# totgokhung123/Event-Retrival-In-Video-Learning-Transferable-Visual-Model-From-Supervised-Natural-Language

Measured on AMD Instinct MI355X. Metric: frames/sec embedded+ranked, ViT-B/32 224², 1/2/4/8 MI355X; R@1/5/10 parity, higher is better.
Workload: dtype bf16; 1 GPU; ViT-B/32 bf16, 10000 frames/GPU x 32 text queries, top-10 (BASELINE configs[1]); frames_per_gpu=10000, global_frames=10000, queries=32, k=10, image_chunk=10000, parallelism=dp1

## Files before the change

### event-retrival-in-video-learning-transferable-visual-model-from-supervised-natural-language_amd/csrc/api.cpp

```cpp
#include <hip/hip_runtime.h>

#include <cmath>
#include <cstdarg>
#include <cstdlib>
#include <cstdio>
#include <cstring>
#include <algorithm>
#include <functional>
#include <memory>
#include <mutex>
#include <string>
#include <system_error>
#include <thread>
#include <vector>

#include "../../include/miclip.h"
#include "src_hash.h"
#include "internal.hpp"

using namespace miclip;

namespace {

thread_local std::string g_err;
// ... 1405 lines not shown

int mi_op_split2h(const float* x, int64_t ldx, int64_t rows, int32_t K, int32_t role, int32_t gelu, void* out,
                  float* scale, void* stream) {
  if (!x || !out || !scale || rows < 0 || role < 0 || role > 2 || (gelu & ~1))
    return fail(MI_ERR_ARG, "mi_op_split2h: bad arguments");
  if (K < 4 || K > 4096 || K % 4 || ldx < K || ldx % 4)
    return fail(MI_ERR_UNSUPPORTED, "mi_op_split2h: 4 <= K <= 4096, K %% 4 == 0, ldx >= K, ldx %% 4 == 0");
  HIP_TRY(split2h_rows(x, ldx, rows, K, role, gelu, (uint16_t*)out, scale, (hipStream_t)stream));
  return MI_OK;
}

int mi_op_gemm_split2h(const void* A3, const void* W3, const float* a_scale, const float* w_scale, const float* bias,
                       float* out, int32_t M, int32_t N, int32_t K3, int32_t epi, void* stream) {
  const int dup = (epi >> 8) & 1;
  epi &= ~0x100;
  if (!A3 || !W3 || !a_scale || !w_scale || !out || M < 0 || N < 1 || K3 < 1 || (epi != EPI_F32 && epi != EPI_RESID_F32))
    return fail(MI_ERR_ARG, "mi_op_gemm_split2h: bad arguments");
  if (N % 128 || K3 % 32) return fail(MI_ERR_UNSUPPORTED, "mi_op_gemm_split2h: N %% 128 == 0, K3 %% 32 == 0");
  GemmArgs g = gargs((const uint16_t*)A3, dup ? 2 * (K3 / 3) : K3, (const uint16_t*)W3, K3, bias, out, N, M, N, K3);
  g.variant = 0;
  g.a_f16 = 1;
  g.rsc = a_scale;
  g.csc = w_scale;
  g.a_dup = dup ? K3 / 3 : 0;
  if (dup && (K3 % 3 || !bias || !gemm_8q_ok(g)))
    return fail(MI_ERR_UNSUPPORTED, "mi_op_gemm_split2h: the [x1 x2] layout needs M >= 256, N %% 256 == 0, K %% 64 == 0");
  HIP_TRY(gemm_bf16(g, epi, (hipStream_t)stream));
  return MI_OK;
}

int mi_op_attention_f32_split(const float* qkv, const float* rmax, float bw, float bb, void* out, int32_t role,
                              float* scale, int32_t B, int32_t S, int32_t W, int32_t causal, void* stream) {
  if (!qkv || !rmax || !out || !scale || B < 0 || S < 1 || W < 64 || (causal & ~1) || (role != 0 && role != 2))
    return fail(MI_ERR_ARG, "mi_op_attention_f32_split: bad arguments");
  if (W % 64 || S > 64) return fail(MI_ERR_UNSUPPORTED, "mi_op_attention_f32_split: W %% 64 == 0 and S <= 64");
  HIP_TRY(attention_f32_split(qkv, rmax, bw, bb, (uint16_t*)out, role, scale, B, S, W, causal, (hipStream_t)stream));
  return MI_OK;
}

int mi_op_attention_f32(const float* qkv, float* out, int32_t B, int32_t S, int32_t W, int32_t causal, void* stream) {
  if (!qkv || !out || B < 0 || S < 1 || W < 64 || (causal & ~1)) return fail(MI_ERR_ARG, "mi_op_attention_f32: bad arguments");
  if (W % 64) return fail(MI_ERR_UNSUPPORTED, "mi_op_attention_f32: W %% 64 == 0");
  HIP_TRY(attention_f32(qkv, out, B, S, W, causal, (hipStream_t)stream));
  return MI_OK;
}

int mi_op_residual_stats(void* x, const void* delta, float* rs, int32_t rows, int32_t W, void* stream) {
  if (!x || !delta || !rs || rows < 0) return fail(MI_ERR_ARG, "mi_op_residual_stats: bad arguments");
  if (W % 4 || W > 1024) return fail(MI_ERR_UNSUPPORTED, "mi_op_residual_stats: W must be a multiple of 4, <= 1024");
  HIP_TRY(residual_stats((float*)x, (const uint16_t*)delta, rs, rows, W, (hipStream_t)stream));
  return MI_OK;
}

int mi_op_gemm_ln(const void* x16, int64_t lda, const float* rs, const void* wf, const float* colsum,
                  const float* colc, void* out, int32_t M, int32_t N, int32_t K, int32_t gelu, void* stream) {
  if (!x16 || !rs || !wf || !colsum || !colc || !out || M < 0 || (gelu & ~1))
    return fail(MI_ERR_ARG, "mi_op_gemm_ln: bad arguments");
  if (M == 0) return MI_OK;
  GemmArgs g = gargs((const uint16_t*)x16, lda, (const uint16_t*)wf, K, colc, out, N, M, N, K);
  g.variant = 0;
  g.a_f16 = 1;
  g.rs = rs;
  g.colv = colsum;
  if (lda < K || lda % 8 || !gemm_8q_ok(g))
    return fail(MI_ERR_UNSUPPORTED, "mi_op_gemm_ln: needs N %% 256 == 0, K %% 128 == 0, K >= 256, M >= 256, "
                                    "lda >= K with lda %% 8 == 0");
  HIP_TRY(gemm_bf16(g, gelu ? EPI_LN_GELU_BF16 : EPI_LN_BF16, (hipStream_t)stream));
  return MI_OK;
}

int mi_op_gemm_residual(void* x16, int64_t ldx, const void* A, int64_t lda, const void* w, const float* bias,
                        float* ps, float* rs, int32_t M, int32_t W, int32_t K, void* stream) {
  if (!x16 || !A || !w || !ps || !rs || M < 0) return fail(MI_ERR_ARG, "mi_op_gemm_residual: bad arguments");
  if (M == 0) return MI_OK;
  GemmArgs g = gargs((const uint16_t*)A, lda, (const uint16_t*)w, K, bias, x16, ldx, M, W, K);
  g.ps = ps;
  if (lda < K || lda % 8 || ldx < W || ldx % 8 || W > 1024 || ((uintptr_t)x16 & 15) || !gemm_8q_ok(g))
    return fail(MI_ERR_UNSUPPORTED, "mi_op_gemm_residual: needs W %% 256 == 0, W <= 1024, K %% 128 == 0, K >= 256, "
                                    "M >= 256, lda >= K and ldx >= W multiples of 8, x16 16-byte aligned");
  HIP_TRY(gemm_bf16(g, EPI_RES16_BF16, (hipStream_t)stream));
  HIP_TRY(residual_finalize(ps, rs, M, W, (hipStream_t)stream));
  return MI_OK;
}

int mi_op_attention(const void* qkv, void* out, int32_t B, int32_t S, int32_t W, int32_t causal, void* stream) {
  if (!qkv || !out || B < 0 || S < 1) return fail(MI_ERR_ARG, "mi_op_attention: bad arguments");
  if (W % 64 || S > 640 || (causal & ~(ATT_CAUSAL | ATT_ONE_WAVE | ATT_STREAM))) return fail(MI_ERR_UNSUPPORTED, "mi_op_attention: W %% 64 == 0 and S <= 640");
  if ((causal & ATT_ONE_WAVE) && !MICLIP_AB) return fail(MI_ERR_UNSUPPORTED, "mi_op_attention: the one-wave kernel (bit 8) is in the A/B build");
  HIP_TRY(attention((const uint16_t*)qkv, (uint16_t*)out, B, S, W, causal, (hipStream_t)stream));
  return MI_OK;
}

int mi_op_gemm_mx(const void* A, const void* a_scale, const void* W, const void* w_scale, const float* bias, void* out,
                  int32_t M, int32_t N, int32_t K, int32_t epi, void* stream) {
  if (!A || !W || !a_scale || !w_scale || !out || M < 0) return fail(MI_ERR_ARG, "mi_op_gemm_mx: bad arguments");
  if (K % 128 || N % 256 || K <= 0) return fail(MI_ERR_UNSUPPORTED, "mi_op_gemm_mx: needs K %% 128 == 0, N %% 256 == 0");
  const int variant = epi >> 8;
  if (variant && !MICLIP_AB) return fail(MI_ERR_UNSUPPORTED, "mi_op_gemm_mx: kernel overrides need the A/B build (make ab)");
  epi &= 0xff;
  if (epi != 0 && epi != 1 && epi != 3 && epi != 4)
    return fail(MI_ERR_ARG, "mi_op_gemm_mx: epilogue 0 (bf16), 1 (GELU), 3 (f32) or 4 (GELU -> MX-fp8)");
  GemmArgs g = gargs((const uint16_t*)A, K, (const uint16_t*)W, K, bias, out, N, M, N, K);
  g.variant = variant;
  g.a_scale = (const uint8_t*)a_scale;
  g.w_scale = (const uint8_t*)w_scale;
  if (epi == 4) g.o_scale = (uint8_t*)out + ((int64_t)M * N + 255) / 256 * 256;
  HIP_TRY(gemm_mx(g, epi, (hipStream_t)stream));
  return MI_OK;
}

int mi_op_quantize_mx(const void* in, void* q, void* scales, int32_t rows, int32_t K, void* stream) {
  if (!in || !q || !scales || rows < 0) return fail(MI_ERR_ARG, "mi_op_quantize_mx: bad arguments");
  if (K % 128 || K <= 0) return fail(MI_ERR_UNSUPPORTED, "mi_op_quantize_mx: K %% 128 == 0");
  HIP_TRY(quantize_mx((const uint16_t*)in, K, (uint8_t*)q, K, (uint8_t*)scales, rows, K, (hipStream_t)stream));
  return MI_OK;
}

int mi_resample_coeffs(int32_t in_size, double in0, double in1, int32_t out_size, int filter, int32_t* kk,
                       int64_t kk_cap, int32_t* bounds) {
  if (!kk || !bounds || in_size < 1 || out_size < 1 || (filter != MI_RESAMPLE_BICUBIC && filter != MI_RESAMPLE_BILINEAR))
    return fail(MI_ERR_ARG, "mi_resample_coeffs: bad arguments");
  std::vector<int32_t> k, b;
  const int ks = resample_coeffs(in_size, in0, in1, out_size, filter, k, b);
  if (ks < 0) return fail(MI_ERR_ARG, "mi_resample_coeffs: bad arguments");
  if ((int64_t)k.size() > kk_cap) return fail(MI_ERR_ARG, "mi_resample_coeffs: kk needs %zu entries", k.size());
  memcpy(kk, k.data(), k.size() * 4);
  memcpy(bounds, b.data(), b.size() * 4);
  return ks;
}

size_t mi_preprocess_workspace_bytes(int64_t B, int32_t H, int32_t W, int32_t n, int mode) {
  return preprocess_workspace_bytes(B, H, W, n, mode);
}

int mi_preprocess_frames(const uint8_t* frames, int64_t B, int32_t H, int32_t W, int32_t n, int mode, void* out,
                         int out_dtype, void* workspace, size_t workspace_bytes, void* stream) {
  if (B < 0 || H < 1 || W < 1 || n < 1 || n > 4096) return fail(MI_ERR_ARG, "mi_preprocess_frames: bad sizes");
  if (mode != MI_PREP_CLIP && mode != MI_PREP_SQUASH) return fail(MI_ERR_ARG, "mi_preprocess_frames: bad mode");
  if (out_dtype != MI_F32 && out_dtype != MI_BF16) return fail(MI_ERR_ARG, "mi_preprocess_frames: out_dtype f32/bf16");
  if (B == 0) return MI_OK;
// ... 115 lines not shown
```

### event-retrival-in-video-learning-transferable-visual-model-from-supervised-natural-language_amd/csrc/attention.hip

```cpp
#include <algorithm>
#include <cstdlib>
#include <type_traits>

#include "common.hpp"
#include "internal.hpp"

namespace miclip {

namespace {


typedef short s16x4 __attribute__((ext_vector_type(4)));
typedef short s16x8 __attribute__((ext_vector_type(8)));

template <int V>
using Int = std::integral_constant<int, V>;

constexpr float sl2 = 0.125f * 1.4426950408889634f;
constexpr float RESCALE = 8.0f;

template <bool P16 = true>
__device__ __forceinline__ float group_max(float v) {
  if (P16) {
    const auto a = __builtin_amdgcn_permlane16_swap(__float_as_uint(v), __float_as_uint(v), false, false);
// ... 314 lines not shown
      }
      const float mu = m[t];
      float ps[4];
#pragma unroll
      for (int kt = 0; kt < 4; ++kt) {
#pragma unroll
        for (int j = 0; j < 4; ++j) sc[kt][j] = __builtin_amdgcn_exp2f(fmaf(sc[kt][j], sl2, -mu));
        ps[kt] = (sc[kt][0] + sc[kt][1]) + (sc[kt][2] + sc[kt][3]);
      }
      l[t] += (ps[0] + ps[1]) + (ps[2] + ps[3]);
      if (SLOTS == 1) {
        __builtin_amdgcn_sched_barrier(0);
        read_vf();
        if (VB) asm volatile("s_waitcnt lgkmcnt(0)" ::: "memory");
      }
#pragma unroll
      for (int s = 0; s < 2; ++s) {
        if (s == 1 && kvalid <= 32) break;
        bf16x8 pb;
#pragma unroll
        for (int j = 0; j < 4; ++j) {
          pb[j] = (__bf16)sc[2 * s][j];
          pb[4 + j] = (__bf16)sc[2 * s + 1][j];
        }
#pragma unroll
        for (int dt = 0; dt < 4; ++dt) o[t][dt] = __builtin_amdgcn_mfma_f32_16x16x32_bf16(vf[dt][s], pb, o[t][dt], 0, 0, 0);
      }
    }
    if (SLOTS > 1 && c + 1 < nch) FA_STAGE_WRITE(slot ^ 1);
    __syncthreads();
  }
#undef FA_STAGE_LOAD
#undef FA_STAGE_WRITE

#pragma unroll
  for (int t = 0; t < NT; ++t) {
    const int qt = wave + NW * t;
    if (qt >= nqt) continue;
    AttnOut{out, q8, qs, rows_pad, bseq, S, W, h}.store16(qt * 16 + fr, g, o[t], 1.0f / group_sum(l[t]));
  }
  if (!PIPE) break;
  item += (int)gridDim.x;
  if (item >= items) break;
  first = false;
  }
}

template <int NT, int PP, int SLOTS = 2>
__global__ __launch_bounds__(512) void attention_flash_kernel(const uint16_t* __restrict__ qkv,
                                                                uint16_t* __restrict__ out, int S, int W, int H,
                                                                int causal, uint8_t* __restrict__ q8,
                                                                uint8_t* __restrict__ qs, int64_t rows_pad) {
  attention_flash_body<NT, PP, SLOTS>(qkv, out, S, W, H, causal, q8, qs, rows_pad);
}

#if MICLIP_AB
__global__ __launch_bounds__(256) __attribute__((amdgpu_waves_per_eu(6))) void attention_short_kernel(
    const uint16_t* __restrict__ qkv, uint16_t* __restrict__ out, int S, int W, int H, int causal,
    uint8_t* __restrict__ q8, uint8_t* __restrict__ qs, int64_t rows_pad) {
  attention_flash_body<1, 2, 1>(qkv, out, S, W, H, causal, q8, qs, rows_pad);
}

__global__ __launch_bounds__(256) void attention_pipe_kernel(const uint16_t* __restrict__ qkv, uint16_t* __restrict__ out,
                                                             int S, int W, int H, int causal, uint8_t* __restrict__ q8,
                                                             uint8_t* __restrict__ qs, int64_t rows_pad, int items) {
  attention_flash_body<1, 2, 1, 1, true>(qkv, out, S, W, H, causal, q8, qs, rows_pad, items);
}

__global__ __launch_bounds__(256) void attention_vb_kernel(const uint16_t* __restrict__ qkv, uint16_t* __restrict__ out,
                                                           int S, int W, int H, int causal, uint8_t* __restrict__ q8,
                                                           uint8_t* __restrict__ qs, int64_t rows_pad) {
  attention_flash_body<1, 2, 1, 1, false, true>(qkv, out, S, W, H, causal, q8, qs, rows_pad);
}

__global__ __launch_bounds__(512) __attribute__((amdgpu_waves_per_eu(6))) void attention_short2_kernel(
    const uint16_t* __restrict__ qkv, uint16_t* __restrict__ out, int S, int W, int H, int causal,
    uint8_t* __restrict__ q8, uint8_t* __restrict__ qs, int64_t rows_pad) {
  attention_flash_body<1, 2, 1, 2>(qkv, out, S, W, H, causal, q8, qs, rows_pad);
}
#endif


template <int NW, bool TT2 = true, bool SPLIT = false, bool SFIRST = false, bool QPF = false>
__global__ __launch_bounds__(NW * 64) void attention_res_kernel(const uint16_t* __restrict__ qkv,
                                                                uint16_t* __restrict__ out, int S, int W, int H,
                                                                uint8_t* __restrict__ q8, uint8_t* __restrict__ qs,
                                                                int64_t rows_pad) {
  extern __shared__ __attribute__((aligned(16))) char res_lds[];
  const int spad = (S + 31) & ~31;
  char* Kimg = res_lds;
  char* Vimg = res_lds + spad * 128;
  const int item = blockIdx.x;
  const int bseq = item / H, h = item % H;
  const int tid = threadIdx.x, lane = tid & 63;
  const int wave = __builtin_amdgcn_readfirstlane(tid >> 6);
  const int64_t ld = 3 * (int64_t)W;
  const uint16_t* qb = qkv + (int64_t)bseq * S * ld + h * 64;
  const uint16_t* kb = qb + W;
  const uint16_t* vb = qb + 2 * W;

  {
    const int nr8 = spad >> 3;
    const int slot = lane & 7;
    for (int i = wave; i < 2 * nr8; i += NW) {
      const bool isv = i >= nr8;
      const int i8 = isv ? i - nr8 : i;
// ... 483 lines not shown
      case 3:
        return launch_kernel(attention_short_kernel, items, 256, s, qkv, out, S, W, H, causal, q8, qs, rows_pad);
      case 1:
        if (!causal)
          return launch_kernel<attention_res_kernel<4, false>>(items, 256, res_lds, s, qkv, out, S, W, H, q8, qs, rows_pad);
        break;
      default: break;
    }
  }
#endif

  if (!one_wave && !stream && !causal && S > 64) {
    int var = ab_env_int("MICLIP_ATTN_VAR", 0);
    if (var < 1 || var > 14) var = S > 320 ? 5 : 1;
    const int vr = S - 16 * ((S + 15) / 16 - 1);
    if (var == 11 || ((var == 12 || var == 13) && !(vr <= 4 && !q8))) var = 1;
    auto res = [&](auto k, int threads, size_t lds) {
      return launch_kernel<decltype(k)::value>(items, threads, lds, s, qkv, out, S, W, H, q8, qs, rows_pad);
    };
    auto r32 = [&](auto k, int threads, int stagger_ticks) {
      return launch_kernel<decltype(k)::value>(items, threads, res_lds, s, qkv, out, S, W, H, q8, qs, rows_pad,
                                               stagger_ticks);
    };
    switch (var) {
      case 1: return res(Kern<attention_res_kernel<8, false>>{}, 512, res_lds);
      case 5: return r32(Kern<attention_r32_kernel<12, false>>{}, 768, 0);
#if MICLIP_AB
      case 2: return res(Kern<attention_res_kernel<8, true>>{}, 512, res_lds);
      case 3: return res(Kern<attention_res_kernel<16, false>>{}, 1024, res_lds);
      case 4: return r32(Kern<attention_r32_kernel<8, true>>{}, 512, 0);
      case 6:
      case 7:
        return r32(Kern<attention_r32_kernel<12, false>>{}, 768, (var - 5) * (S * S / 378));
      case 8: return r32(Kern<attention_r32_kernel<12, false, 2>>{}, 768, 0);
      case 10: return r32(Kern<attention_r32_kernel<12, false, 0, true>>{}, 768, 0);
      case 12: return res(Kern<attention_res_kernel<8, false, true>>{}, 512, res_lds + (size_t)8 * vr * 68 * 4);
      case 13: return res(Kern<attention_res_kernel<8, false, true, true>>{}, 512, res_lds + (size_t)8 * vr * 68 * 4);
      case 14: return res(Kern<attention_res_kernel<8, false, false, false, true>>{}, 512, res_lds);
      default: return r32(Kern<attention_r32_kernel<12, false, 1>>{}, 768, 0);
#else
      default: return hipErrorNotSupported;
#endif
    }
  }

#if MICLIP_AB
  if (one_wave)
    return with_value<32, 64, 96>(std::max(32, (S + 31) & ~31), [&](auto sp) {
      return launch_kernel(attention_kernel<decltype(sp)::value>, items, 64, s, qkv, out, S, W, H, causal, items);
    });
#endif

  const int nqt = (S + 15) / 16;
  if (nqt <= 4)
    return launch_kernel(attention_flash_kernel<1, 2, 1>, items, 256, s, qkv, out, S, W, H, causal | q0, q8, qs, rows_pad);
  return with_value<1, 2, 3, 4, 5>((nqt + 7) / 8, [&](auto nt) {
    return launch_kernel(attention_flash_kernel<decltype(nt)::value, 1>, items, 512, s, qkv, out, S, W, H, causal, q8, qs,
                         rows_pad);
  });
}

}
```

### event-retrival-in-video-learning-transferable-visual-model-from-supervised-natural-language_amd/csrc/encoder.hip

```cpp
#include <cstdlib>

#include "common.hpp"
#include "internal.hpp"

namespace miclip {

namespace {

constexpr float LN_EPS = 1e-5f;

struct RowVals {
  float4 v[4];
};

__device__ __forceinline__ void ln_stats(RowVals& r, int n4, int lane, int W, float& mean, float& rstd) {
  float s = 0.f;
#pragma unroll
  for (int i = 0; i < 4; ++i)
    if (lane + 64 * i < n4) s += (r.v[i].x + r.v[i].y) + (r.v[i].z + r.v[i].w);
  mean = wave_sum(s) / (float)W;
  float ss = 0.f;
#pragma unroll
  for (int i = 0; i < 4; ++i)
    if (lane + 64 * i < n4) {
// ... 108 lines not shown
  float mean, rstd;
  ln_stats(r, n4, lane, W, mean, rstd);
  ln_store(r, mean, rstd, g, b, out + (int64_t)row * W, q, qs, row, (rows + 1) & ~1, lane, n4);
}

__global__ __launch_bounds__(256) void vision_embed_ln_kernel(float* __restrict__ x, const float* __restrict__ cls,
                                                              const float* __restrict__ pos, const float* __restrict__ g,
                                                              const float* __restrict__ b, int rows, int S, int W,
                                                              const float* __restrict__ g1,
                                                              const float* __restrict__ b1, uint16_t* __restrict__ h) {
  const int row = blockIdx.x * 4 + (threadIdx.x >> 6), lane = threadIdx.x & 63;
  if (row >= rows) return;
  const int t = row % S, n4 = W >> 2;
  float4* xr = (float4*)(x + (int64_t)row * W);
  const float4* src = t == 0 ? (const float4*)cls : (const float4*)xr;
  const float4* p4 = (const float4*)(pos + (int64_t)t * W);
  RowVals r;
#pragma unroll
  for (int i = 0; i < 4; ++i) {
    const int idx = lane + 64 * i;
    if (idx < n4) {
      const float4 s = src[idx], p = p4[idx];
      r.v[i] = make_float4(s.x + p.x, s.y + p.y, s.z + p.z, s.w + p.w);
    } else {
      r.v[i] = make_float4(0.f, 0.f, 0.f, 0.f);
    }
  }
  float mean, rstd;
  ln_stats(r, n4, lane, W, mean, rstd);
  const float4* g4 = (const float4*)g;
  const float4* b4 = (const float4*)b;
#pragma unroll
  for (int i = 0; i < 4; ++i) {
    const int idx = lane + 64 * i;
    if (idx < n4) {
      const float4 gg = g4[idx], bb = b4[idx];
      r.v[i] = make_float4((r.v[i].x - mean) * rstd * gg.x + bb.x, (r.v[i].y - mean) * rstd * gg.y + bb.y,
                           (r.v[i].z - mean) * rstd * gg.z + bb.z, (r.v[i].w - mean) * rstd * gg.w + bb.w);
      xr[idx] = r.v[i];
    }
  }
  if (h) {
    ln_stats(r, n4, lane, W, mean, rstd);
    ln_store(r, mean, rstd, g1, b1, h + (int64_t)row * W, nullptr, nullptr, row, 0, lane, n4);
  }
}

__device__ __forceinline__ void store_row_stats(RowVals& r, int n4, int lane, int W, float* rs, int row) {
  float mean, rstd;
  ln_stats(r, n4, lane, W, mean, rstd);
  if (lane == 0) *(float2*)(rs + 2 * (int64_t)row) = make_float2(rstd, rstd * mean);
}

__global__ __launch_bounds__(256) void vision_embed_ln16_kernel(float* __restrict__ x, const float* __restrict__ cls,
                                                                const float* __restrict__ pos,
                                                                const float* __restrict__ g,
                                                                const float* __restrict__ b, int rows, int S, int W,
                                                                float* __restrict__ rs) {
  typedef _Float16 h4v __attribute__((ext_vector_type(4)));
  const int row = blockIdx.x * 4 + (threadIdx.x >> 6), lane = threadIdx.x & 63;
  if (row >= rows) return;
  const int t = row % S, n4 = W >> 2;
  const float4* xr = (const float4*)(x + (int64_t)row * W);
  h4v* xh = (h4v*)((_Float16*)x + (int64_t)row * W * 2);
  const float4* src = t == 0 ? (const float4*)cls : xr;
  const float4* p4 = (const float4*)(pos + (int64_t)t * W);
  RowVals r;
#pragma unroll
  for (int i = 0; i < 4; ++i) {
    const int idx = lane + 64 * i;
    if (idx < n4) {
      const float4 sv = src[idx], p = p4[idx];
      r.v[i] = make_float4(sv.x + p.x, sv.y + p.y, sv.z + p.z, sv.w + p.w);
    } else {
      r.v[i] = make_float4(0.f, 0.f, 0.f, 0.f);
    }
  }
  float mean, rstd;
  ln_stats(r, n4, lane, W, mean, rstd);
  const float4* g4 = (const float4*)g;
  const float4* b4 = (const float4*)b;
#pragma unroll
  for (int i = 0; i < 4; ++i) {
    const int idx = lane + 64 * i;
    if (idx < n4) {
      const float4 gg = g4[idx], bb = b4[idx];
      const h4v o{(_Float16)((r.v[i].x - mean) * rstd * gg.x + bb.x), (_Float16)((r.v[i].y - mean) * rstd * gg.y + bb.y),
                  (_Float16)((r.v[i].z - mean) * rstd * gg.z + bb.z), (_Float16)((r.v[i].w - mean) * rstd * gg.w + bb.w)};
      r.v[i] = make_float4((float)o[0], (float)o[1], (float)o[2], (float)o[3]);
      xh[idx] = o;
    }
  }
  store_row_stats(r, n4, lane, W, rs, row);
}

__global__ __launch_bounds__(256) void residual_stats_kernel(float* __restrict__ x, const uint16_t* __restrict__ delta,
                                                             float* __restrict__ rs, int rows, int W) {
  typedef _Float16 h4v __attribute__((ext_vector_type(4)));
  typedef uint32_t u2v __attribute__((ext_vector_type(2)));
  const int row = blockIdx.x * 4 + (threadIdx.x >> 6), lane = threadIdx.x & 63;
  if (row >= rows) return;
  const int n4 = W >> 2;
  h4v* xh = (h4v*)((_Float16*)x + (int64_t)row * W * 2);
  const u2v* dr = (const u2v*)(delta + (int64_t)row * W);
  RowVals r;
#pragma unroll
  for (int i = 0; i < 4; ++i) {
    const int idx = lane + 64 * i;
    if (idx < n4) {
      const h4v vh = __builtin_nontemporal_load(&xh[idx]);
      const u2v d = __builtin_nontemporal_load(&dr[idx]);
      const h4v o{(_Float16)((float)vh[0] + bf2f((uint16_t)(d[0] & 0xffff))),
                  (_Float16)((float)vh[1] + bf2f((uint16_t)(d[0] >> 16))),
                  (_Float16)((float)vh[2] + bf2f((uint16_t)(d[1] & 0xffff))),
                  (_Float16)((float)vh[3] + bf2f((uint16_t)(d[1] >> 16)))};
      __builtin_nontemporal_store(o, &xh[idx]);
      r.v[i] = make_float4((float)o[0], (float)o[1], (float)o[2], (float)o[3]);
    } else {
      r.v[i] = make_float4(0.f, 0.f, 0.f, 0.f);
    }
  }
  store_row_stats(r, n4, lane, W, rs, row);
}

__global__ __launch_bounds__(256) void residual_finalize_kernel(const float* __restrict__ ps, float* __restrict__ rs,
                                                                int rows, int W) {
  __shared__ float4 sp[256 * 8 + 256 / 4];
  const int np = W >> 6, nq = np >> 1;
  const int r0 = blockIdx.x * 256;
  const int nrow = min(256, rows - r0);
  const float4* src = (const float4*)(ps + (int64_t)r0 * np * 2);
  for (int i = threadIdx.x; i < nrow * nq; i += 256) {
    const int r = i / nq;
    sp[i + (r >> 2)] = src[i];
  }
  __syncthreads();
  const int row = r0 + threadIdx.x;
  if (row >= rows) return;
  const float4* p4 = sp + threadIdx.x * nq + (threadIdx.x >> 2);
  float s[16], m2[16];
#pragma unroll
  for (int i = 0; i < 8; ++i)
    if (i < nq) {
// ... 142 lines not shown
      }
    }
    packed[e >> 1] = (uint32_t)f2bf(v[0]) | ((uint32_t)f2bf(v[1]) << 16);
  }
  *(uint4*)(out + prow * Kp + kb) = make_uint4(packed[0], packed[1], packed[2], packed[3]);
}

__global__ __launch_bounds__(256) void finalize_kernel(const float* __restrict__ y, void* __restrict__ out,
                                                       int out_dtype, int rows, int D, int l2) {
  const int row = blockIdx.x * 4 + (threadIdx.x >> 6), lane = threadIdx.x & 63;
  if (row >= rows) return;
  const float* yr = y + (int64_t)row * D;
  float inv = 1.f;
  if (l2) {
    float ss = 0.f;
    for (int c = lane; c < D; c += 64) ss += yr[c] * yr[c];
    const float n = sqrtf(wave_sum(ss));
    inv = (l2 == 2 && !(n > 1e-8f)) ? 1.0f : 1.0f / n;
  }
  for (int c = lane; c < D; c += 64) {
    const float v = l2 ? yr[c] * inv : yr[c];
    if (out_dtype == 0) ((float*)out)[(int64_t)row * D + c] = v;
    else if (out_dtype == 1) ((uint16_t*)out)[(int64_t)row * D + c] = f2bf(v);
    else ((_Float16*)out)[(int64_t)row * D + c] = (_Float16)v;
  }
}

}

hipError_t layernorm_bf16(const float* x, int64_t in_stride, const float* g, const float* b, uint16_t* out,
                          int64_t out_stride, int rows, int W, hipStream_t s, uint8_t* q, uint8_t* qs) {
  if (rows <= 0) return hipSuccess;
  if (W % 4 || W > 1024 || (q && W % 128)) return hipErrorInvalidValue;
  hipLaunchKernelGGL(ln_bf16_kernel, dim3((rows + 3) / 4), dim3(256), 0, s, x, in_stride, g, b, out, out_stride,
                     rows, W, q, qs);
  return hipGetLastError();
}

hipError_t vision_embed_ln(float* x, const float* cls, const float* pos, const float* g, const float* b, int B,
                           int S, int W, hipStream_t s, const float* g1, const float* b1, uint16_t* h) {
  const int rows = B * S;
  if (rows <= 0) return hipSuccess;
  if (W % 4 || W > 1024) return hipErrorInvalidValue;
  hipLaunchKernelGGL(vision_embed_ln_kernel, dim3((rows + 3) / 4), dim3(256), 0, s, x, cls, pos, g, b, rows, S, W,
                     g1, b1, h);
  return hipGetLastError();
}

hipError_t vision_embed_ln16(float* x, const float* cls, const float* pos, const float* g, const float* b, int B,
                             int S, int W, float* rs, hipStream_t s) {
  const int rows = B * S;
  if (W % 4 || W > 1024) return hipErrorInvalidValue;
  if (rows <= 0) return hipSuccess;
  hipLaunchKernelGGL(vision_embed_ln16_kernel, dim3((rows + 3) / 4), dim3(256), 0, s, x, cls, pos, g, b, rows, S, W, rs);
  return hipGetLastError();
}

hipError_t residual_stats(float* x, const uint16_t* delta, float* rs, int rows, int W, hipStream_t s) {
  if (W % 4 || W > 1024) return hipErrorInvalidValue;
  if (rows <= 0) return hipSuccess;
  hipLaunchKernelGGL(residual_stats_kernel, dim3((rows + 3) / 4), dim3(256), 0, s, x, delta, rs, rows, W);
  return hipGetLastError();
}

hipError_t residual_finalize(const float* ps, float* rs, int rows, int W, hipStream_t s) {
  if (W % 128 || W > 1024 || W <= 0) return hipErrorInvalidValue;
  if (rows <= 0) return hipSuccess;
  hipLaunchKernelGGL(residual_finalize_kernel, dim3((rows + 255) / 256), dim3(256), 0, s, ps, rs, rows, W);
  return hipGetLastError();
}

hipError_t text_embed(const int32_t* tokens, const float* tok_emb, const float* pos, float* x, int Q, int S, int W,
                      int vocab, hipStream_t s) {
  const int64_t total4 = (int64_t)Q * S * (W / 4);
  if (total4 <= 0) return hipSuccess;
  hipLaunchKernelGGL(text_embed_kernel, dim3((unsigned)((total4 + 255) / 256)), dim3(256), 0, s, tokens, tok_emb,
                     pos, x, total4, S, W, vocab);
  return hipGetLastError();
}

hipError_t eot_gather_ln(const int32_t* tokens, const float* x, const uint16_t* delta, const float* g,
                         const float* b, uint16_t* out, int Q, int S, int W, hipStream_t s) {
  if (Q <= 0) return hipSuccess;
  hipLaunchKernelGGL(eot_gather_ln_kernel, dim3((Q + 3) / 4), dim3(256), 0, s, tokens, x, delta, g, b, out, Q, S,
                     W);
  return hipGetLastError();
}

hipError_t residual_ln(float* x, const uint16_t* delta, int64_t stride, int write_x, const float* g, const float* b,
                       uint16_t* out, int rows, int W, hipStream_t s, uint8_t* q, uint8_t* qs, int xmode) {
  if (rows <= 0) return hipSuccess;
  if (W % 4 || W > 1024 || (q && W % 128) || xmode < RES_F32 || xmode > RES_F16) return hipErrorInvalidValue;
#if MICLIP_AB
  static int nts = -1;
  if (nts < 0) {
    const char* e = getenv("MICLIP_LN_NT");
    nts = e ? atoi(e) : 1;
  }
#else
  constexpr int nts = 1;
#endif
  const dim3 grid((rows + 3) / 4), block(256);
#define RLN(NT, XM) hipLaunchKernelGGL((residual_ln_kernel<NT, XM>), grid, block, 0, s, x, delta, stride, write_x, g, b, out, rows, W, q, qs)
  if (nts) {
    if (xmode == RES_F32) RLN(true, RES_F32);
    else if (xmode == RES_F32_TO_F16) RLN(true, RES_F32_TO_F16);
    else RLN(true, RES_F16);
  } else {
// ... 35 lines not shown
```

### event-retrival-in-video-learning-transferable-visual-model-from-supervised-natural-language_amd/miclip/_native.py

```python
from __future__ import annotations

import ctypes
import os

import numpy as np

from .config import CLIPConfig

LIB_NAME = "libmiclip.so"
LIB_PATH = os.path.join(os.path.dirname(os.path.abspath(__file__)), LIB_NAME)
CSRC_DIR = os.path.join(os.path.dirname(os.path.dirname(os.path.abspath(__file__))), "csrc")
AB_LIB_PATH = os.path.join(os.path.dirname(os.path.dirname(os.path.dirname(os.path.abspath(__file__)))),
                           "scripts", "ab", "libmiclip_ab.so")

MI_F32, MI_BF16, MI_F16, MI_FP8 = 0, 1, 2, 3
MI_NAN_FIRST, MI_NAN_LAST = 0, 1
MI_NORM_L2, MI_NORM_L2_GUARD, MI_NORM_NONE = 0, 1, 2
MI_PREP_CLIP, MI_PREP_SQUASH = 0, 1
MI_RESAMPLE_BICUBIC, MI_RESAMPLE_BILINEAR = 0, 1

EXPORTS = (
    "mi_abi_version", "mi_build_id", "mi_build_sources", "mi_last_error", "mi_clip_weights_numel", "mi_clip_create", "mi_clip_destroy",
    "mi_clip_reserve", "mi_clip_encode_image", "mi_clip_encode_text", "mi_rank_workspace_bytes",
    "mi_rank_topk", "mi_rank_merge", "mi_score_matrix", "mi_rank_of_targets",
    "mi_op_gemm", "mi_op_gemm_f32", "mi_op_layernorm", "mi_op_attention", "mi_op_residual_ln",
    "mi_op_residual_stats", "mi_op_gemm_ln", "mi_op_gemm_residual", "mi_op_split6",
    "mi_resample_coeffs", "mi_preprocess_workspace_bytes", "mi_preprocess_frames",
    "mi_jpeg_workspace_bytes", "mi_jpeg_decode", "mi_host_gather",
    "mi_op_quantize_mx", "mi_op_gemm_mx",
    "mi_mirror_build", "mi_rank_mirror_workspace_bytes", "mi_rank_mirror", "mi_normalize_rows_f16",
    "mi_jpeg_decode_transform", "mi_op_split2h", "mi_op_gemm_split2h", "mi_op_attention_f32",
    "mi_op_attention_f32_split",
    "mi_clip_kernel_events", "mi_clip_kernel_times",
    "mi_rank_filtered_workspace_bytes", "mi_rank_topk_filtered",
    "mi_rank_collapse_workspace_bytes", "mi_rank_collapse",
)


class MiClipError(RuntimeError):
    pass


class Arch(ctypes.Structure):
    _fields_ = [(n, ctypes.c_int32) for n in (
        "embed_dim", "image_resolution", "vision_layers", "vision_width", "vision_patch_size",
        "context_length", "vocab_size", "text_width", "text_heads", "text_layers")]

    @classmethod
    def from_config(cls, cfg: CLIPConfig) -> "Arch":
        return cls(cfg.embed_dim, cfg.image_resolution, cfg.vision_layers, cfg.vision_width,
                   cfg.vision_patch_size, cfg.context_length, cfg.vocab_size, cfg.text_width,
                   cfg.text_heads, cfg.text_layers)


_lib = None
_lib_ab = None


def lib():
    global _lib
    if _lib is not None:
        return _lib
    if os.environ.get("MICLIP_LIB") == "ab":
        _lib = lib_ab()
        return _lib
    if not os.path.isfile(LIB_PATH):
        raise MiClipError(f"{LIB_PATH} not found: build it with `python -c 'import __graft_entry__ as g; g.build()'`"
                          " or `make -C <pkg>/csrc`")
    _lib = _bind(LIB_PATH)
    return _lib


def lib_ab():
    global _lib_ab
    if _lib_ab is not None:
        return _lib_ab
    if not os.path.isfile(AB_LIB_PATH):
        raise MiClipError(f"{AB_LIB_PATH} not found: `make -C <pkg>/csrc ab`")
    _lib_ab = _bind(AB_LIB_PATH)
    return _lib_ab


def _bind(path):
    import torch
    L = ctypes.CDLL(path)
    P, I32, I64, SZ = ctypes.c_void_p, ctypes.c_int32, ctypes.c_int64, ctypes.c_size_t
    sig = {
        "mi_abi_version": (ctypes.c_int, []),
        "mi_build_id": (ctypes.c_char_p, []),
        "mi_build_sources": (ctypes.c_char_p, []),
        "mi_last_error": (ctypes.c_char_p, []),
        "mi_clip_weights_numel": (I64, [ctypes.POINTER(Arch)]),
        "mi_clip_create": (ctypes.c_int, [ctypes.POINTER(Arch), P, I64, ctypes.c_int, ctypes.c_int,
                                          ctypes.POINTER(P)]),
        "mi_clip_destroy": (ctypes.c_int, [P]),
        "mi_clip_reserve": (ctypes.c_int, [P, I64, I64]),
        "mi_clip_encode_image": (ctypes.c_int, [P, P, I64, ctypes.c_int, P, ctypes.c_int, ctypes.c_int, P]),
        "mi_clip_encode_text": (ctypes.c_int, [P, P, I64, P, ctypes.c_int, ctypes.c_int, P]),
        "mi_rank_workspace_bytes": (SZ, [I64, I64, I32]),
        "mi_rank_topk": (ctypes.c_int, [P, I64, I64, ctypes.c_int, P, I64, I32, I64, ctypes.c_int, ctypes.c_int,
                                        P, P, P, SZ, P]),
        "mi_rank_merge": (ctypes.c_int, [P, P, I64, I64, I32, ctypes.c_int, P, P, P]),
        "mi_rank_filtered_workspace_bytes": (SZ, [I64, I64, I32]),
        "mi_rank_topk_filtered": (ctypes.c_int, [P, I64, I64, ctypes.c_int, P, I64, I32, I64, ctypes.c_int,
                                                 ctypes.c_int, P, P, P, P, P, SZ, P]),
        "mi_rank_collapse_workspace_bytes": (SZ, [I64, I32, I64]),
        "mi_rank_collapse": (ctypes.c_int, [P, I64, ctypes.c_int, P, I64, ctypes.c_int, I64, I64, P, P, I64, I32,
                                            I32, ctypes.c_float, P, P, P, P, P, SZ, P]),
        "mi_mirror_build": (ctypes.c_int, [P, I64, I64, ctypes.c_int, P, P]),
        "mi_rank_mirror_workspace_bytes": (SZ, [I64, I64]),
        "mi_normalize_rows_f16": (ctypes.c_int, [P, I64, I64, P, P]),
        "mi_rank_mirror": (ctypes.c_int, [P, P, I64, I64, ctypes.c_int, P, I64, I32, I64, ctypes.c_int, P, P, P, P,
                                          SZ, P]),
        "mi_score_matrix": (ctypes.c_int, [P, I64, I64, ctypes.c_int, P, I64, ctypes.c_int, P, P]),
        "mi_rank_of_targets": (ctypes.c_int, [P, I64, I64, P, P, I64, P, P]),
        "mi_op_gemm": (ctypes.c_int, [P, P, P, P, I32, I32, I32, I32, P]),
        "mi_op_gemm_f32": (ctypes.c_int, [P, P, P, P, I32, I32, I32, I32, P]),
        "mi_op_layernorm": (ctypes.c_int, [P, P, P, P, I32, I32, P]),
        "mi_op_attention": (ctypes.c_int, [P, P, I32, I32, I32, I32, P]),
        "mi_op_residual_ln": (ctypes.c_int, [P, P, P, P, P, I32, I32, I32, P]),
        "mi_op_residual_stats": (ctypes.c_int, [P, P, P, I32, I32, P]),
        "mi_op_gemm_ln": (ctypes.c_int, [P, I64, P, P, P, P, P, I32, I32, I32, I32, P]),
        "mi_op_gemm_residual": (ctypes.c_int, [P, I64, P, I64, P, P, P, P, I32, I32, I32, P]),
        "mi_op_split6": (ctypes.c_int, [P, I64, I64, I32, I32, I32, P, P]),
        "mi_op_split2h": (ctypes.c_int, [P, I64, I64, I32, I32, I32, P, P, P]),
        "mi_op_gemm_split2h": (ctypes.c_int, [P, P, P, P, P, P, I32, I32, I32, I32, P]),
        "mi_op_attention_f32": (ctypes.c_int, [P, P, I32, I32, I32, I32, P]),
        "mi_op_attention_f32_split": (ctypes.c_int, [P, P, ctypes.c_float, ctypes.c_float, P, I32, P, I32, I32, I32, I32,
                                                     P]),
        "mi_clip_kernel_events": (ctypes.c_int, [P, I32, I32]),
        "mi_clip_kernel_times": (ctypes.c_int, [P, P, I32]),
        "mi_op_quantize_mx": (ctypes.c_int, [P, P, P, I32, I32, P]),
        "mi_op_gemm_mx": (ctypes.c_int, [P, P, P, P, P, P, I32, I32, I32, I32, P]),
        "mi_resample_coeffs": (ctypes.c_int, [I32, ctypes.c_double, ctypes.c_double, I32, ctypes.c_int, P, I64, P]),
        "mi_preprocess_workspace_bytes": (SZ, [I64, I32, I32, I32, ctypes.c_int]),
        "mi_preprocess_frames": (ctypes.c_int, [P, I64, I32, I32, I32, ctypes.c_int, P, ctypes.c_int, P, SZ, P]),
        "mi_jpeg_workspace_bytes": (SZ, [P, I32, I64]),
        "mi_jpeg_decode": (ctypes.c_int, [P, I64, P, P, P, P, I32, P, P, I32, P, P, SZ, P]),
        "mi_jpeg_decode_transform": (ctypes.c_int, [P, I64, P, P, P, P, I32, P, P, I32, I32, ctypes.c_int, P,
                                                    ctypes.c_int, P, SZ, P]),
        "mi_host_gather": (ctypes.c_int, [P, P, P, I64, I32]),
    }
    for name, (res, args) in sig.items():
        fn = getattr(L, name)
        fn.restype = res
        fn.argtypes = args
    if L.mi_abi_version() != 7:
        raise MiClipError("libmiclip ABI version mismatch")
    _check_sources(L, path)
    return L


def source_fingerprint(names, csrc=None):
    import hashlib
    csrc = csrc or CSRC_DIR
    h = hashlib.sha256()
    for n in names:
        with open(os.path.join(csrc, n), "rb") as f:
            h.update(f.read())
    return h.hexdigest()[:16]


def _check_sources(L, path):
    if not os.path.isdir(CSRC_DIR):
        return
    names = L.mi_build_sources().decode().split()
    missing = [n for n in names if not os.path.isfile(os.path.join(CSRC_DIR, n))]
    if missing:
        raise MiClipError(f"{path}: built from sources missing here ({', '.join(missing)}); rebuild with build()")
    built, here = L.mi_build_id().decode(), source_fingerprint(names)
    if built != here:
        raise MiClipError(f"{path} was built from other sources (fingerprint {built}) than {CSRC_DIR} ({here}): "
                          "rebuild with `python -c 'import __graft_entry__ as g; g.build()'` or `make -C <pkg>/csrc`")

# ... 48 lines not shown
```

### include/miclip.h

```cpp
#ifndef MICLIP_H
#define MICLIP_H

#include <stddef.h>
#include <stdint.h>

#ifdef __cplusplus
extern "C" {
#endif

#define MICLIP_ABI_VERSION 7

enum mi_dtype { MI_F32 = 0, MI_BF16 = 1, MI_F16 = 2, MI_FP8 = 3  };
enum mi_status { MI_OK = 0, MI_ERR_ARG = -1, MI_ERR_HIP = -2, MI_ERR_UNSUPPORTED = -3, MI_ERR_STATE = -4 };
enum mi_nan_policy { MI_NAN_FIRST = 0, MI_NAN_LAST = 1 };
enum mi_norm_mode {
  MI_NORM_L2 = 0,
  MI_NORM_L2_GUARD = 1,
  MI_NORM_NONE = 2
};

enum mi_prep_mode {
  MI_PREP_CLIP = 0,
  MI_PREP_SQUASH = 1
};
// ... 60 lines not shown
                     void* workspace, size_t workspace_bytes, void* stream);

int mi_mirror_build(const void* corpus, int64_t N, int64_t D, int corpus_dtype, void* mirror_f16, void* stream);

int mi_normalize_rows_f16(const void* rows, int64_t N, int64_t D, void* out, void* stream);

size_t mi_rank_mirror_workspace_bytes(int64_t N, int64_t Q);

int mi_rank_mirror(const void* mirror_f16, const void* master, int64_t N, int64_t D, int master_dtype,
                   const float* queries, int64_t Q, int32_t k, int64_t index_base, int nan_policy,
                   float* out_scores, int64_t* out_index, int32_t* out_certified,
                   void* workspace, size_t workspace_bytes, void* stream);

int mi_rank_merge(const float* cand_scores, const int64_t* cand_index, int64_t Q, int64_t C,
                  int32_t k, int nan_policy, float* out_scores, int64_t* out_index, void* stream);

int mi_score_matrix(const void* corpus, int64_t N, int64_t D, int corpus_dtype,
                    const float* queries, int64_t Q, int norm_mode, float* out, void* stream);

int mi_rank_of_targets(const float* scores, int64_t Q, int64_t N, const int64_t* pair_query,
                       const int64_t* pair_target, int64_t T, int64_t* out_rank, void* stream);

int mi_resample_coeffs(int32_t in_size, double in0, double in1, int32_t out_size, int filter, int32_t* kk,
                       int64_t kk_cap, int32_t* bounds);

size_t mi_preprocess_workspace_bytes(int64_t B, int32_t H, int32_t W, int32_t n, int mode);

int mi_preprocess_frames(const uint8_t* frames, int64_t B, int32_t H, int32_t W, int32_t n, int mode, void* out,
                         int out_dtype, void* workspace, size_t workspace_bytes, void* stream);

#define MI_JPEG_HUFF_BYTES 3480
size_t mi_jpeg_workspace_bytes(const int32_t* geom, int32_t B, int64_t data_bytes);
int mi_jpeg_decode(const uint8_t* data, int64_t data_bytes, const int64_t* seg_off, const int64_t* seg_end, const void* huff,
                   const int32_t* huff_idx, int32_t nsets, const uint16_t* qtab, const int32_t* geom, int32_t B,
                   uint8_t* out_rgb, void* workspace, size_t workspace_bytes, void* stream);

int mi_jpeg_decode_transform(const uint8_t* data, int64_t data_bytes, const int64_t* seg_off, const int64_t* seg_end,
                             const void* huff, const int32_t* huff_idx, int32_t nsets, const uint16_t* qtab,
                             const int32_t* geom, int32_t B, int32_t n, int mode, void* out, int out_dtype,
                             void* workspace, size_t workspace_bytes, void* stream);

int mi_host_gather(void* dst, const void* const* src, const int64_t* len, int64_t n, int32_t threads);

int mi_op_gemm(const void* A, const void* W, const float* bias, void* out, int32_t M, int32_t N, int32_t K,
               int32_t epilogue, void* stream);
int mi_op_gemm_f32(const float* A, const float* W, const float* bias, float* out, int32_t M, int32_t N, int32_t K,
                   int32_t epilogue, void* stream);
int mi_op_layernorm(const float* x, const float* gamma, const float* beta, void* out, int32_t rows, int32_t W,
                    void* stream);
int mi_op_attention(const void* qkv, void* out, int32_t B, int32_t S, int32_t W, int32_t causal, void* stream);
int mi_op_residual_ln(void* x, const void* delta, const float* gamma, const float* beta, void* out, int32_t rows,
                      int32_t W, int32_t xmode, void* stream);
int mi_op_residual_stats(void* x, const void* delta, float* rs, int32_t rows, int32_t W, void* stream);
int mi_op_split6(const float* x, int64_t ldx, int64_t rows, int32_t K, int32_t role, int32_t gelu, void* out,
                 void* stream);
int mi_op_split2h(const float* x, int64_t ldx, int64_t rows, int32_t K, int32_t role, int32_t gelu, void* out,
                  float* scale, void* stream);
enum mi_kernel_kind { MI_KERNEL_NONE = 0, MI_KERNEL_C_FC = 1 };
int mi_clip_kernel_events(mi_clip* ctx, int32_t kind, int32_t capacity);
int mi_clip_kernel_times(mi_clip* ctx, float* us, int32_t n);
int mi_op_gemm_split2h(const void* A3, const void* W3, const float* a_scale, const float* w_scale, const float* bias,
                       float* out, int32_t M, int32_t N, int32_t K3, int32_t epi, void* stream);
int mi_op_attention_f32(const float* qkv, float* out, int32_t B, int32_t S, int32_t W, int32_t causal, void* stream);
int mi_op_attention_f32_split(const float* qkv, const float* rmax, float bw, float bb, void* out, int32_t role,
                              float* scale, int32_t B, int32_t S, int32_t W, int32_t causal, void* stream);
int mi_op_gemm_ln(const void* x16, int64_t lda, const float* rs, const void* Wf, const float* colsum,
                  const float* colc, void* out, int32_t M, int32_t N, int32_t K, int32_t gelu, void* stream);
int mi_op_gemm_residual(void* x16, int64_t ldx, const void* A, int64_t lda, const void* W, const float* bias,
                        float* ps, float* rs, int32_t M, int32_t Wd, int32_t K, void* stream);

int mi_op_quantize_mx(const void* in, void* q, void* scales, int32_t rows, int32_t K, void* stream);
int mi_op_gemm_mx(const void* A, const void* a_scale, const void* W, const void* w_scale, const float* bias, void* out,
                  int32_t M, int32_t N, int32_t K, int32_t epi, void* stream);

#ifdef __cplusplus
}
#endif
#endif
```

Baseline: 120,100 frames/s.

## Add single-query-row attention kernel for last layer and nontemporal embed-LN

Adds a dedicated attention kernel for the case where only the CLS query row is needed (q0, short sequences). One wave per head computes scores against all keys, does the softmax and P·V with MFMA, and writes only row 0, instead of running the full flash kernel over every query tile. It also switches the vision embed+LayerNorm kernel to nontemporal loads and stores to avoid cache pollution, and exposes that op through the API. The work saved is limited to the last layer's attention, which is a small share of the whole ViT encoder.

```diff
diff --git a/event-retrival-in-video-learning-transferable-visual-model-from-supervised-natural-language_amd/csrc/api.cpp b/event-retrival-in-video-learning-transferable-visual-model-from-supervised-natural-language_amd/csrc/api.cpp
--- a/event-retrival-in-video-learning-transferable-visual-model-from-supervised-natural-language_amd/csrc/api.cpp
+++ b/event-retrival-in-video-learning-transferable-visual-model-from-supervised-natural-language_amd/csrc/api.cpp
@@ -1481,6 +1481,14 @@
   return MI_OK;
 }
 
+int mi_op_vision_embed_ln16(void* x, const float* cls, const float* pos, const float* gamma, const float* beta,
+                            float* rs, int32_t B, int32_t S, int32_t W, void* stream) {
+  if (!x || !cls || !pos || !gamma || !beta || !rs || B < 0 || S < 1) return fail(MI_ERR_ARG, "mi_op_vision_embed_ln16: bad arguments");
+  if (W % 4 || W > 1024) return fail(MI_ERR_UNSUPPORTED, "mi_op_vision_embed_ln16: W must be a multiple of 4, <= 1024");
+  HIP_TRY(vision_embed_ln16((float*)x, cls, pos, gamma, beta, B, S, W, rs, (hipStream_t)stream));
+  return MI_OK;
+}
+
 int mi_op_gemm_ln(const void* x16, int64_t lda, const float* rs, const void* wf, const float* colsum,
                   const float* colc, void* out, int32_t M, int32_t N, int32_t K, int32_t gelu, void* stream) {
   if (!x16 || !rs || !wf || !colsum || !colc || !out || M < 0 || (gelu & ~1))
@@ -1514,7 +1522,7 @@
 
 int mi_op_attention(const void* qkv, void* out, int32_t B, int32_t S, int32_t W, int32_t causal, void* stream) {
   if (!qkv || !out || B < 0 || S < 1) return fail(MI_ERR_ARG, "mi_op_attention: bad arguments");
-  if (W % 64 || S > 640 || (causal & ~(ATT_CAUSAL | ATT_ONE_WAVE | ATT_STREAM))) return fail(MI_ERR_UNSUPPORTED, "mi_op_attention: W %% 64 == 0 and S <= 640");
+  if (W % 64 || S > 640 || (causal & ~(ATT_CAUSAL | ATT_ONE_WAVE | ATT_STREAM | ATT_Q0_ONLY))) return fail(MI_ERR_UNSUPPORTED, "mi_op_attention: W %% 64 == 0 and S <= 640");
   if ((causal & ATT_ONE_WAVE) && !MICLIP_AB) return fail(MI_ERR_UNSUPPORTED, "mi_op_attention: the one-wave kernel (bit 8) is in the A/B build");
   HIP_TRY(attention((const uint16_t*)qkv, (uint16_t*)out, B, S, W, causal, (hipStream_t)stream));
   return MI_OK;
diff --git a/event-retrival-in-video-learning-transferable-visual-model-from-supervised-natural-language_amd/csrc/attention.hip b/event-retrival-in-video-learning-transferable-visual-model-from-supervised-natural-language_amd/csrc/attention.hip
--- a/event-retrival-in-video-learning-transferable-visual-model-from-supervised-natural-language_amd/csrc/attention.hip
+++ b/event-retrival-in-video-learning-transferable-visual-model-from-supervised-natural-language_amd/csrc/attention.hip
@@ -390,6 +390,122 @@
                                                                 int causal, uint8_t* __restrict__ q8,
                                                                 uint8_t* __restrict__ qs, int64_t rows_pad) {
   attention_flash_body<NT, PP, SLOTS>(qkv, out, S, W, H, causal, q8, qs, rows_pad);
+}
+
+__global__ __launch_bounds__(256) void attention_q0_kernel(const uint16_t* __restrict__ qkv, uint16_t* __restrict__ out,
+                                                           int S, int W, int H, int items) {
+  constexpr int VS = 68;
+  __shared__ __attribute__((aligned(16))) uint16_t Vsh[4][64 * VS];
+  const int lane = threadIdx.x & 63, wave = threadIdx.x >> 6;
+  const int item = blockIdx.x * 4 + wave;
+  if (item >= items) return;
+  uint16_t* Vs = Vsh[wave];
+  const int bseq = item / H, h = item % H;
+  const int64_t ld = 3 * (int64_t)W;
+  const uint16_t* qb = qkv + (int64_t)bseq * S * ld + h * 64;
+  const uint16_t* kb = qb + W;
+  const uint16_t* vb = qb + 2 * W;
+  const int fr = lane & 15, g = lane >> 4, fk = 8 * g;
+  const int kvalid = S;
+
+  bf16x8 kf[4][2], qf[2], vf[4][2];
+  uint4 vr[8];
+#pragma unroll
+  for (int kt = 0; kt < 4; ++kt) {
+    const int r = kt * 16 + fr;
+#pragma unroll
+    for (int s = 0; s < 2; ++s) {
+      uint4 k = make_uint4(0, 0, 0, 0);
+      if (r < S) k = *(const uint4*)(kb + (int64_t)r * ld + 32 * s + fk);
+      kf[kt][s] = __builtin_bit_cast(bf16x8, k);
+    }
+  }
+#pragma unroll
+  for (int i = 0; i < 8; ++i) {
+    const int r = i * 8 + (lane >> 3), ch = lane & 7;
+    vr[i] = make_uint4(0, 0, 0, 0);
+    if (r < S) vr[i] = *(const uint4*)(vb + (int64_t)r * ld + ch * 8);
+  }
+#pragma unroll
+  for (int s = 0; s < 2; ++s) qf[s] = *(const bf16x8*)(qb + 32 * s + fk);
+#pragma unroll
+  for (int i = 0; i < 8; ++i) {
+    const int r = i * 8 + (lane >> 3), ch = lane & 7;
+    const uint16_t* vv = (const uint16_t*)&vr[i];
+#pragma unroll
+    for (int e = 0; e < 8; ++e) Vs[(ch * 8 + e) * VS + r] = vv[e];
+  }
+
+  float m = -INFINITY, l = 0.f;
+  f32x4 o[4];
+#pragma unroll
+  for (int dt = 0; dt < 4; ++dt) o[dt] = f32x4{0.f, 0.f, 0.f, 0.f};
+  f32x4 sc[4];
+#pragma unroll
+  for (int kt = 0; kt < 4; ++kt) {
+    f32x4 acc = {0.f, 0.f, 0.f, 0.f};
+    if (kt * 16 < kvalid) {
+#pragma unroll
+      for (int s = 0; s < 2; ++s) acc = __builtin_amdgcn_mfma_f32_16x16x32_bf16(kf[kt][s], qf[s], acc, 0, 0, 0);
+    }
+    sc[kt] = acc;
+  }
+  if (kvalid < 64) {
+#pragma unroll
+    for (int kt = 0; kt < 4; ++kt)
+#pragma unroll
+      for (int j = 0; j < 4; ++j) {
+        const int key = kt * 16 + 4 * g + j;
+        if (key >= S) sc[kt][j] = -INFINITY;
+      }
+  }
+  float cm = fmaxf(fmaxf(fmaxf(sc[0][0], sc[0][1]), fmaxf(sc[0][2], sc[0][3])),
+                   fmaxf(fmaxf(sc[1][0], sc[1][1]), fmaxf(sc[1][2], sc[1][3])));
+  cm = fmaxf(cm, fmaxf(fmaxf(fmaxf(sc[2][0], sc[2][1]), fmaxf(sc[2][2], sc[2][3])),
+                       fmaxf(fmaxf(sc[3][0], sc[3][1]), fmaxf(sc[3][2], sc[3][3]))));
+  cm = group_max(cm);
+  const float cmu = cm * sl2;
+  if (cmu > m + RESCALE) {
+    const float alpha = __builtin_amdgcn_exp2f(m - cmu);
+    l *= alpha;
+#pragma unroll
+    for (int dt = 0; dt < 4; ++dt) o[dt] *= alpha;
+    m = cmu;
+  }
+  const float mu = m;
+  float ps[4];
+#pragma unroll
+  for (int kt = 0; kt < 4; ++kt) {
+#pragma unroll
+    for (int j = 0; j < 4; ++j) sc[kt][j] = __builtin_amdgcn_exp2f(fmaf(sc[kt][j], sl2, -mu));
+    ps[kt] = (sc[kt][0] + sc[kt][1]) + (sc[kt][2] + sc[kt][3]);
+  }
+  l += (ps[0] + ps[1]) + (ps[2] + ps[3]);
+  asm volatile("s_waitcnt lgkmcnt(0)" ::: "memory");
+  __builtin_amdgcn_wave_barrier();
+#pragma unroll
+  for (int dt = 0; dt < 4; ++dt)
+#pragma unroll
+    for (int s = 0; s < 2; ++s) {
+      const uint16_t* vrow = &Vs[(dt * 16 + fr) * VS + 32 * s + 4 * g];
+      const uint2 lo = *(const uint2*)vrow;
+      const uint2 hi = *(const uint2*)(vrow + 16);
+      vf[dt][s] = __builtin_bit_cast(bf16x8, make_uint4(lo.x, lo.y, hi.x, hi.y));
+    }
+#pragma unroll
+  for (int s = 0; s < 2; ++s) {
+    if (s == 1 && kvalid <= 32) break;
+    bf16x8 pb;
+#pragma unroll
+    for (int j = 0; j < 4; ++j) {
+      pb[j] = (__bf16)sc[2 * s][j];
+      pb[4 + j] = (__bf16)sc[2 * s + 1][j];
+    }
+#pragma unroll
+    for (int dt = 0; dt < 4; ++dt) o[dt] = __builtin_amdgcn_mfma_f32_16x16x32_bf16(vf[dt][s], pb, o[dt], 0, 0, 0);
+  }
+  const float inv = 1.0f / group_sum(l);
+  if (fr == 0) AttnOut{out, nullptr, nullptr, 0, bseq, S, W, h}.row16_bf16(0, g, o, inv);
 }
 
 #if MICLIP_AB
@@ -979,6 +1095,8 @@
 #endif
 
   const int nqt = (S + 15) / 16;
+  if (nqt <= 4 && q0 && !causal && !q8 && ab_env_int("MICLIP_ATTN_Q0", 1) != 0)
+    return launch_kernel(attention_q0_kernel, (items + 3) / 4, 256, s, qkv, out, S, W, H, items);
   if (nqt <= 4)
     return launch_kernel(attention_flash_kernel<1, 2, 1>, items, 256, s, qkv, out, S, W, H, causal | q0, q8, qs, rows_pad);
   return with_value<1, 2, 3, 4, 5>((nqt + 7) / 8, [&](auto nt) {
diff --git a/event-retrival-in-video-learning-transferable-visual-model-from-supervised-natural-language_amd/csrc/encoder.hip b/event-retrival-in-video-learning-transferable-visual-model-from-supervised-natural-language_amd/csrc/encoder.hip
--- a/event-retrival-in-video-learning-transferable-visual-model-from-supervised-natural-language_amd/csrc/encoder.hip
+++ b/event-retrival-in-video-learning-transferable-visual-model-from-supervised-natural-language_amd/csrc/encoder.hip
@@ -184,12 +184,14 @@
   if (lane == 0) *(float2*)(rs + 2 * (int64_t)row) = make_float2(rstd, rstd * mean);
 }
 
+template <bool NTS>
 __global__ __launch_bounds__(256) void vision_embed_ln16_kernel(float* __restrict__ x, const float* __restrict__ cls,
                                                                 const float* __restrict__ pos,
                                                                 const float* __restrict__ g,
                                                                 const float* __restrict__ b, int rows, int S, int W,
                                                                 float* __restrict__ rs) {
   typedef _Float16 h4v __attribute__((ext_vector_type(4)));
+  typedef float f4v __attribute__((ext_vector_type(4)));
   const int row = blockIdx.x * 4 + (threadIdx.x >> 6), lane = threadIdx.x & 63;
   if (row >= rows) return;
   const int t = row % S, n4 = W >> 2;
@@ -202,7 +204,14 @@
   for (int i = 0; i < 4; ++i) {
     const int idx = lane + 64 * i;
     if (idx < n4) {
-      const float4 sv = src[idx], p = p4[idx];
+      float4 sv;
+      if (NTS) {
+        const f4v v = __builtin_nontemporal_load((const f4v*)src + idx);
+        sv = make_float4(v[0], v[1], v[2], v[3]);
+      } else {
+        sv = src[idx];
+      }
+      const float4 p = p4[idx];
       r.v[i] = make_float4(sv.x + p.x, sv.y + p.y, sv.z + p.z, sv.w + p.w);
     } else {
       r.v[i] = make_float4(0.f, 0.f, 0.f, 0.f);
@@ -220,7 +229,8 @@
       const h4v o{(_Float16)((r.v[i].x - mean) * rstd * gg.x + bb.x), (_Float16)((r.v[i].y - mean) * rstd * gg.y + bb.y),
                   (_Float16)((r.v[i].z - mean) * rstd * gg.z + bb.z), (_Float16)((r.v[i].w - mean) * rstd * gg.w + bb.w)};
       r.v[i] = make_float4((float)o[0], (float)o[1], (float)o[2], (float)o[3]);
-      xh[idx] = o;
+      if (NTS) __builtin_nontemporal_store(o, &xh[idx]);
+      else xh[idx] = o;
     }
   }
   store_row_stats(r, n4, lane, W, rs, row);
@@ -469,8 +479,12 @@
   const int rows = B * S;
   if (W % 4 || W > 1024) return hipErrorInvalidValue;
   if (rows <= 0) return hipSuccess;
-  hipLaunchKernelGGL(vision_embed_ln16_kernel, dim3((rows + 3) / 4), dim3(256), 0, s, x, cls, pos, g, b, rows, S, W, rs);
-  return hipGetLastError();
+  const dim3 grid((rows + 3) / 4);
+#if MICLIP_AB
+  if (ab_env_int("MICLIP_EMBED_NT", 1) == 0)
+    return launch_kernel(vision_embed_ln16_kernel<false>, grid, 256, s, x, cls, pos, g, b, rows, S, W, rs);
+#endif
+  return launch_kernel(vision_embed_ln16_kernel<true>, grid, 256, s, x, cls, pos, g, b, rows, S, W, rs);
 }
 
 hipError_t residual_stats(float* x, const uint16_t* delta, float* rs, int rows, int W, hipStream_t s) {
diff --git a/event-retrival-in-video-learning-transferable-visual-model-from-supervised-natural-language_amd/miclip/_native.py b/event-retrival-in-video-learning-transferable-visual-model-from-supervised-natural-language_amd/miclip/_native.py
--- a/event-retrival-in-video-learning-transferable-visual-model-from-supervised-natural-language_amd/miclip/_native.py
+++ b/event-retrival-in-video-learning-transferable-visual-model-from-supervised-natural-language_amd/miclip/_native.py
@@ -24,7 +24,7 @@
     "mi_clip_reserve", "mi_clip_encode_image", "mi_clip_encode_text", "mi_rank_workspace_bytes",
     "mi_rank_topk", "mi_rank_merge", "mi_score_matrix", "mi_rank_of_targets",
     "mi_op_gemm", "mi_op_gemm_f32", "mi_op_layernorm", "mi_op_attention", "mi_op_residual_ln",
-    "mi_op_residual_stats", "mi_op_gemm_ln", "mi_op_gemm_residual", "mi_op_split6",
+    "mi_op_residual_stats", "mi_op_vision_embed_ln16", "mi_op_gemm_ln", "mi_op_gemm_residual", "mi_op_split6",
     "mi_resample_coeffs", "mi_preprocess_workspace_bytes", "mi_preprocess_frames",
     "mi_jpeg_workspace_bytes", "mi_jpeg_decode", "mi_host_gather",
     "mi_op_quantize_mx", "mi_op_gemm_mx",
@@ -120,6 +120,7 @@
         "mi_op_attention": (ctypes.c_int, [P, P, I32, I32, I32, I32, P]),
         "mi_op_residual_ln": (ctypes.c_int, [P, P, P, P, P, I32, I32, I32, P]),
         "mi_op_residual_stats": (ctypes.c_int, [P, P, P, I32, I32, P]),
+        "mi_op_vision_embed_ln16": (ctypes.c_int, [P, P, P, P, P, P, I32, I32, I32, P]),
         "mi_op_gemm_ln": (ctypes.c_int, [P, I64, P, P, P, P, P, I32, I32, I32, I32, P]),
         "mi_op_gemm_residual": (ctypes.c_int, [P, I64, P, I64, P, P, P, P, I32, I32, I32, P]),
         "mi_op_split6": (ctypes.c_int, [P, I64, I64, I32, I32, I32, P, P]),
diff --git a/include/miclip.h b/include/miclip.h
--- a/include/miclip.h
+++ b/include/miclip.h
@@ -136,6 +136,8 @@
 int mi_op_residual_ln(void* x, const void* delta, const float* gamma, const float* beta, void* out, int32_t rows,
                       int32_t W, int32_t xmode, void* stream);
 int mi_op_residual_stats(void* x, const void* delta, float* rs, int32_t rows, int32_t W, void* stream);
+int mi_op_vision_embed_ln16(void* x, const float* cls, const float* pos, const float* gamma, const float* beta,
+                            float* rs, int32_t B, int32_t S, int32_t W, void* stream);
 int mi_op_split6(const float* x, int64_t ldx, int64_t rows, int32_t K, int32_t role, int32_t gelu, void* out,
                  void* stream);
 int mi_op_split2h(const float* x, int64_t ldx, int64_t rows, int32_t K, int32_t role, int32_t gelu, void* out,
```

Measured after the change: 120,300 frames/s, median of 6. Within noise of the previous version (+0.2%).
